# adamgreig/basebandboard

Hardware: AMD Instinct MI355X
Metric: awgn_clt_gsamples_per_s (higher is better)
Workload: dtype u32 bit-sliced GF(2) / int8 out

## Files before the change

### basebandboard_amd/csrc/awgn_kernels.hip

```cpp
#include "bbb_common.hpp"
#include "bitslice_util.hpp"
#include "awgn_launch.hpp"

#include <cstdlib>
#include <mutex>
#include <type_traits>
#include "gen/lutopt256_gen.inc"

namespace bbb {


template <int W32, typename TabPtr>
__device__ __forceinline__ void nibble_matvec_part(TabPtr tab, int nlo, int nhi, const uint32_t (&x)[W32],
                                                   uint32_t (&y)[W32]) {
    constexpr int C = (W32 % 4 == 0) ? 4 : (W32 % 2 == 0 ? 2 : 1);
    constexpr int NC = W32 / C;
    typedef uint32_t chunk_t __attribute__((ext_vector_type(C)));
#pragma unroll
    for (int w = 0; w < W32; w++) {
        uint32_t xw = x[w];
        asm volatile("" : "+v"(xw));
#pragma unroll
        for (int q = 0; q < 8; q += 2) {
            const int n0 = w * 8 + q, n1 = n0 + 1;
// ... 368 lines not shown


struct TxFuse {
    int16_t coeffs[64];
    const uint32_t *bits;
    uint32_t rel_base;
    uint32_t c0;
    int32_t noise_var;
    int32_t bit_en;
    int32_t use_bits;
    uint32_t last_word;
};

static TxFuse make_txfuse(const int16_t *coeffs, const uint32_t *d_bits, uint32_t nwords32, uint32_t rel_base, uint32_t c0, int noise_var,
                          int bit_en, int use_bits) {
    TxFuse tx;
    for (int i = 0; i < 64; i++) tx.coeffs[i] = coeffs[i];
    tx.bits = d_bits;
    tx.rel_base = rel_base;
    tx.c0 = c0;
    tx.noise_var = noise_var;
    tx.bit_en = bit_en;
    tx.use_bits = use_bits && nwords32 >= 2;
    tx.last_word = nwords32 ? nwords32 - 1 : 1;
    return tx;
}

__device__ __forceinline__ uint32_t bfi_uniform(uint32_t mask, uint32_t a, uint32_t b) {
    uint32_t d;
    asm("v_bfi_b32 %0, %1, %2, %3" : "=v"(d) : "s"(mask), "v"(a), "v"(b));
    return d;
}

typedef uint16_t u16x2 __attribute__((ext_vector_type(2)));
typedef int16_t i16x2 __attribute__((ext_vector_type(2)));

template <bool TX>
__global__ void __launch_bounds__(64) __attribute__((amdgpu_waves_per_eu(1, 1)))
awgn256_kernel(const uint32_t *__restrict planes, void *__restrict dst_, unsigned long long nsamples,
               unsigned L, unsigned long long G, unsigned nlanes, TxFuse tx) {
    __shared__ uint32_t Z[16 * 8 * 64];
    __shared__ __attribute__((aligned(16))) uint16_t TT[TX ? 256 * 8 : 8];
    const unsigned lane = threadIdx.x;
    const unsigned long long wave = blockIdx.x;
    const unsigned long long LG = wave * 64 + lane;
    __builtin_amdgcn_s_setprio(3);

    uint32_t selmask[4] = {0, 0, 0, 0};
    if (TX) {
        for (int e = (int)lane; e < 256 * 8; e += 64) {
            const int q = e >> 3, j = e & 7, ph = (int)((tx.c0 + (unsigned)j) & 7u);
            int sum = 0;
#pragma unroll
            for (int idx = 0; idx < 8; idx++) {
                const int c = tx.coeffs[8 * idx + ph];
                sum += ((q >> (7 - idx)) & 1) ? c : -c;
            }
            const int shaped = tx.bit_en ? ((int)((unsigned)sum << 20) >> 20) : 0;
            TT[e] = (uint16_t)((unsigned)((shaped - 128 * tx.noise_var) * 16) & 0xffffu);
        }
#pragma unroll
        for (int d = 0; d < 4; d++)
            selmask[d] = (tx.c0 + 2u * (unsigned)d < 8u ? 0x0000ffffu : 0u) | (tx.c0 + 2u * (unsigned)d + 1u < 8u ? 0xffff0000u : 0u);
        __syncthreads();
    }

// ... 122 lines not shown
                        if (ii < 3) load_z(4 * ihalf + ii + 1, zn);
                        const uint32_t w4[4] = {win[ii], win[4 + ii], win[8 + ii], win[12 + ii]};
                        round_end(full_c, 4 * ihalf + ii, w4, zc);
                    }
                }
            } else {
                const uint32_t none[4] = {0, 0, 0, 0};
                uint32_t zc[16], zn[16];
                load_z(0, zn);
#pragma unroll 1
                for (unsigned i = 0; i < 8; i++) {
#pragma unroll
                    for (int e = 0; e < 16; e++) zc[e] = zn[e];
                    load_z((i + 1) & 7, zn);
                    round_end(full_c, i, none, zc);
                }
            }
        };
        if (wave_full) all_iterations(std::true_type{});
        else all_iterations(std::false_type{});
    }
}

template <bool SMALL>
__global__ void __launch_bounds__(64) __attribute__((amdgpu_waves_per_eu(1, 1)))
awgn256_planes_kernel(const uint32_t *__restrict planes, u32x4 *__restrict stage, unsigned L, unsigned nlanes
) {
    const unsigned lane = threadIdx.x;
    const unsigned long long wave = blockIdx.x;
    const unsigned long long LG = wave * 64 + lane;
    __builtin_amdgcn_s_setprio(3);
    uint32_t a[256], b[256], pa[256], pb[256], cnt[8];
    if constexpr (SMALL) {
#ifdef BBB_SMALL_THROTTLE
        asm volatile("" ::: BBB_SMALL_THROTTLE);
#endif
        const uint32_t voff = (uint32_t)LG * 4u;
#define BBB_PLANE(p) (*reinterpret_cast<const uint32_t *>(reinterpret_cast<const char *>(planes + (size_t)(p) * nlanes) + (unsigned long long)voff))
#define BBB_PARK(p) { const uint32_t v_ = BBB_PLANE(p); BBB_ACC_WRITE(pa[p], v_); }
        LUTOPT256_FOR_PARKED_HI(BBB_PARK)
#undef BBB_PARK
#pragma unroll
        for (int p = 0; p < 256; p++)
            if (!lutopt256_hi_is_parked(p)) a[p] = BBB_PLANE(p);
#undef BBB_PLANE
    } else {
#pragma unroll
        for (int p = 0; p < 256; p++) b[p] = planes[(size_t)p * nlanes + LG];
        lutopt256_advance(b, a);
#define BBB_PARK(p) BBB_ACC_WRITE(pa[p], a[p]);
        LUTOPT256_FOR_PARKED_HI(BBB_PARK)
#undef BBB_PARK
    }
    u32x4 *out = stage + (wave * L) * 128 + lane;
#pragma unroll 1
    for (unsigned t = 0; t < L; t += 2) {
        lutopt256_step_parked_hi(a, pa, b, pb, cnt);
        {
        __builtin_nontemporal_store((u32x4){cnt[0], cnt[1], cnt[2], cnt[3]}, out);
        __builtin_nontemporal_store((u32x4){cnt[4], cnt[5], cnt[6], cnt[7]}, out + 64);
        }
        lutopt256_step_parked_hi(b, pb, a, pa, cnt);
        {
        __builtin_nontemporal_store((u32x4){cnt[0], cnt[1], cnt[2], cnt[3]}, out + 128);
        __builtin_nontemporal_store((u32x4){cnt[4], cnt[5], cnt[6], cnt[7]}, out + 192);
        }
        out += 256;
    }
}

int awgn256_planes_launch(const uint32_t *d_planes, void *stage, unsigned L, unsigned nlanes, hipStream_t st, bool small_footprint) {
    if (L & 1) return fail(BBB_EINVAL, "segment length must be even");
    if (small_footprint)
        hipLaunchKernelGGL(awgn256_planes_kernel<true>, dim3(nlanes / 64), dim3(64), 0, st, d_planes, (u32x4 *)stage, L, nlanes);
    else
        hipLaunchKernelGGL(awgn256_planes_kernel<false>, dim3(nlanes / 64), dim3(64), 0, st, d_planes, (u32x4 *)stage, L, nlanes);
    BBB_HIP(hipGetLastError());
    return BBB_OK;
}

constexpr unsigned kUnplaneRaw = 32 * 1024, kUnplaneLds = 3 * 32 * 1024, kUnplaneLdsTx = kUnplaneLds + 32 * 1024 + 2 * 2048;

struct UnplaneGeom {
    unsigned w_lo, ngroups, nunits;
    unsigned per_block;
};

template <bool TXM, bool NOWRAP = false>
__global__ void __launch_bounds__(256, 7)
unplane_kernel(const u32x4 *__restrict stage, char *__restrict dst, unsigned long long win_lo, unsigned long long nbytes_, unsigned L,
               unsigned long long G, UnplaneGeom ge, TxFuse tx) {
    extern __shared__ __attribute__((aligned(16))) uint32_t lds[];
    typedef __attribute__((address_space(3))) void *lds_void_ptr;
    const unsigned tid = threadIdx.x, lane = tid & 63;
    const unsigned wv = (unsigned)__builtin_amdgcn_readfirstlane((int)(tid >> 6));
    if (blockIdx.x * ge.per_block >= ge.nunits) return;
    char *const dstw = dst - win_lo;
    const unsigned long long nbytes = win_lo + nbytes_;
    const unsigned l8 = tid & 7, qs = tid >> 3;
    const unsigned wr0 = l8 * 32 + ((((qs >> 2) ^ (2 * ((l8 >> 1) & 3))) << 2) | (qs & 3));
    const unsigned lq = (tid >> 3) & 7, c2 = tid & 7;
    const unsigned rd0 = (wv * 8 + lq) * 32 + ((c2 ^ (2 * ((lq >> 1) & 3))) << 2);
    uint32_t *const tile = lds + 2 * (kUnplaneRaw / 4);
    uint32_t *const T10 = lds + kUnplaneLds / 4;
    uint32_t *const winb = lds + kUnplaneLds / 4 + 8192;
    if (TXM) {
        uint16_t *const TT = reinterpret_cast<uint16_t *>(tile);
        for (int e = (int)tid; e < 256 * 8; e += 256) {
            const int q = e >> 3, j = e & 7, ph = (int)((tx.c0 + (unsigned)j) & 7u);
            int sum = 0;
#pragma unroll
            for (int idx = 0; idx < 8; idx++) {
                const int c = tx.coeffs[8 * idx + ph];
                sum += ((q >> (7 - idx)) & 1) ? c : -c;
            }
            const int shaped = tx.bit_en ? ((int)((unsigned)sum << 20) >> 20) : 0;
            TT[e] = (uint16_t)((unsigned)((shaped - 128 * tx.noise_var) * (NOWRAP ? 1 : 16)) & 0xffffu);
        }
        __syncthreads();
        for (unsigned p = tid; p < 1024 * 8; p += 256) {
            const unsigned q10 = p >> 3, e = 2 * (p & 7);
            const uint32_t lo = TT[(((q10 >> ((tx.c0 + e) >> 3)) & 0xffu) << 3) + (e & 7)];
            const uint32_t hi = TT[(((q10 >> ((tx.c0 + e + 1) >> 3)) & 0xffu) << 3) + ((e + 1) & 7)];
            T10[p] = lo | (hi << 16);
        }
        __syncthreads();
    }
    struct Pos { unsigned q8, rg, w; };
    auto advance = [&](Pos &p) {
        if (++p.rg == ge.ngroups) {
            p.rg = 0;
            if (++p.q8 == 8) { p.q8 = 0; p.w++; }
        }
    };
    const unsigned voff_lane = (lane & 7) * 16 + (lane >> 3) * 8192;
    auto dma_unit = [&](const Pos &p, unsigned buf) {
        const unsigned step0 = p.rg * 128;
        const unsigned long long wabs = (unsigned long long)ge.w_lo + p.w;
        const char *const sb = reinterpret_cast<const char *>(stage) + ((wabs * L + step0) * 128 + p.q8 * 8) * 16;
        uint32_t *const rawb = lds + buf * (kUnplaneRaw / 4) + wv * 8 * 256;
        if (step0 + 128 <= L) {
            const char *const pl = sb + wv * 2048 + voff_lane;
#pragma unroll
            for (unsigned k = 0; k < 8; k++)
                __builtin_amdgcn_global_load_lds((const void *)(pl + ((k & 3) * 32 * 2048 + (k >> 2) * 1024)),
                                                 (lds_void_ptr)(uintptr_t)(rawb + k * 256), 16, 0, 0);
        } else {
            const unsigned last = L - 1 - step0;
#pragma unroll
            for (unsigned k = 0; k < 8; k++) {
                unsigned st = 4 * ((k & 3) * 8 + (lane >> 3)) + wv;
                st = st < last ? st : last;
                __builtin_amdgcn_global_load_lds((const void *)(sb + (size_t)st * 2048 + (k >> 2) * 1024 + (lane & 7) * 16),
                                                 (lds_void_ptr)(uintptr_t)(rawb + k * 256), 16, 0, 0);
            }
        }
        if (TXM) {
            const long long so = (long long)((wabs * 2048 + p.q8 * 8) * (unsigned long long)L + step0) - (long long)win_lo;
#pragma unroll
            for (unsigned i = 0; i < 2; i++) {
                const unsigned e = (wv * 2 + i) * 64 + lane, row = e >> 1;
                const long long pu = so + (long long)((unsigned long long)((row >> 3) * 64 + (row & 7)) * L);
                uint32_t word = 0;
                if (pu > -128 && pu < (long long)nbytes_) word = (((uint32_t)(pu >> 3) + tx.rel_base) >> 5) + (e & 1);
                word = word < tx.last_word ? word : tx.last_word;
                __builtin_amdgcn_global_load_lds((const void *)(tx.bits + word), (lds_void_ptr)(uintptr_t)(winb + buf * 512 + (wv * 2 + i) * 64), 4, 0, 0);
            }
        }
    };
    auto wait_vm = [](unsigned n) {
        switch (n) {
#define BBB_W(N) case N: asm volatile("s_waitcnt vmcnt(" #N ")" ::: "memory"); break;
            BBB_W(8) BBB_W(10) BBB_W(16) BBB_W(26)
#undef BBB_W
        default: asm volatile("s_waitcnt vmcnt(0)" ::: "memory"); break;
        }
    };
    constexpr unsigned NDMA = TXM ? 10 : 8, NST = TXM ? 16 : 8;
    const unsigned u0 = blockIdx.x * ge.per_block;
    const unsigned n_it = ge.nunits - u0 < ge.per_block ? ge.nunits - u0 : ge.per_block;
    Pos cur;
    cur.rg = u0 % ge.ngroups;
    cur.q8 = (u0 / ge.ngroups) & 7;
    cur.w = (u0 / ge.ngroups) >> 3;
    Pos nxt = cur;
    advance(nxt);
    unsigned buf = 0;
    bool fast1 = false;
    dma_unit(cur, 0);
    for (unsigned it = 0; it < n_it; it++, buf ^= 1) {
        const unsigned q8 = cur.q8, step0 = cur.rg * 128;
        const unsigned long long w = (unsigned long long)ge.w_lo + cur.w;
        const bool more1 = it + 1 < n_it;
        if (more1) dma_unit(nxt, buf ^ 1);
        wait_vm((more1 ? NDMA : 0u) + (fast1 ? NST : 0u));
        __builtin_amdgcn_s_barrier();
        {
            const uint32_t *raw = lds + buf * (kUnplaneRaw / 4) + (qs * 8 + l8) * 4;
            uint32_t Z[4][8];
#pragma unroll
            for (unsigned s = 0; s < 4; s++) {
                const u32x4 lo = *reinterpret_cast<const u32x4 *>(raw + (2 * s) * 1024);
                const u32x4 hi = *reinterpret_cast<const u32x4 *>(raw + (2 * s + 1) * 1024);
                Z[s][0] = lo[0]; Z[s][1] = lo[1]; Z[s][2] = lo[2]; Z[s][3] = lo[3];
                Z[s][4] = hi[0]; Z[s][5] = hi[1]; Z[s][6] = hi[2]; Z[s][7] = TXM ? ~hi[3] : hi[3];
            }
#pragma unroll
            for (unsigned s = 0; s < 4; s++) planes8_to_bytes(Z[s]);
#pragma unroll
            for (unsigned i = 0; i < 8; i++) {
                uint32_t z[4] = {Z[0][i], Z[1][i], Z[2][i], Z[3][i]};
                transpose4x4_bytes(z);
#pragma unroll
                for (unsigned q = 0; q < 4; q++) tile[wr0 + (8 * q + i) * 256] = z[q];
            }
        }
        asm volatile("s_waitcnt lgkmcnt(0)" ::: "memory");
        __builtin_amdgcn_s_barrier();
        const unsigned inseg = step0 + c2 * 16;
        const unsigned long long g0 = (w * 32 + wv) * 64 + q8 * 8 + lq;
        unsigned long long off = g0 * (unsigned long long)L + inseg;
        const unsigned long long goff = 256ull * L;
        const bool lane_fast = inseg < L && g0 + 7 * 256 < G && off >= win_lo && off + 7 * goff + 16 <= nbytes;
        const bool wave_fast = __all(lane_fast);
        fast1 = wave_fast;
        if (!TXM && inseg < L) {
            if (wave_fast) {
#pragma unroll
                for (unsigned k = 0; k < 8; k++) {
                    const u32x4 v = *reinterpret_cast<const u32x4 *>(&tile[rd0 + k * 1024]);
                    *reinterpret_cast<u32x4 *>(dstw + off) = v;
                    off += goff;
                }
            } else {
                for (unsigned k = 0; k < 8; k++, off += goff) {
                    if (g0 + 256ull * k >= G || off >= nbytes) break;
                    if (off < win_lo) continue;
                    const u32x4 v = *reinterpret_cast<const u32x4 *>(&tile[rd0 + k * 1024]);
// ... 36 lines not shown
                        x[2 * w4] = __builtin_bit_cast(uint32_t, __builtin_bit_cast(i16x2, m01) >> 4);
                        x[2 * w4 + 1] = __builtin_bit_cast(uint32_t, __builtin_bit_cast(i16x2, m23) >> 4);
                    }
                }
                int16_t *out = dst16 + (o - win_lo);
                if (FULL || o + 16 <= nbytes) {
                    const u32x4 lo = {x[0], x[1], x[2], x[3]}, hi = {x[4], x[5], x[6], x[7]};
                    reinterpret_cast<u32x4 *>(out)[0] = lo;
                    reinterpret_cast<u32x4 *>(out)[1] = hi;
                } else {
                    const unsigned n = (unsigned)(nbytes - o);
                    for (unsigned e = 0; e < n; e++) out[e] = (int16_t)((x[e >> 1] >> (16 * (e & 1))) & 0xffff);
                }
            };
            if (wave_fast) {
#pragma unroll 1
                for (unsigned k4 = 0; k4 < 8; k4 += 4) {
#pragma unroll
                    for (unsigned k = 0; k < 4; k++) piece(std::true_type{}, k4 + k, off + (k4 + k) * goff);
                }
            } else {
#pragma unroll 1
                for (unsigned k = 0; k < 8; k++) {
                    const unsigned long long o = off + k * goff;
                    if (g0 + 256ull * k >= G || o >= nbytes) break;
                    if (o < win_lo) continue;
                    piece(std::false_type{}, k, o);
                }
            }
        }
        asm volatile("s_waitcnt lgkmcnt(0)" ::: "memory");
        __builtin_amdgcn_s_barrier();
        cur = nxt;
        advance(nxt);
    }
}

static bool unplane_tx_nowrap(const TxFuse &tx) {
    int worst = 0;
    if (tx.bit_en)
        for (int ph = 0; ph < 8; ph++) {
            int sum = 0;
            for (int idx = 0; idx < 8; idx++) sum += tx.coeffs[8 * idx + ph] < 0 ? -(int)tx.coeffs[8 * idx + ph] : (int)tx.coeffs[8 * idx + ph];
            worst = sum > worst ? sum : worst;
        }
    return tx.noise_var >= 0 && worst + 128 * tx.noise_var <= 2047;
}

static int unplane_launch_with(const void *stage, void *dst, uint64_t win_lo, uint64_t nbytes, unsigned L, uint64_t G, unsigned nlanes,
                               const TxFuse *tx, hipStream_t st) {
    if (win_lo & 15) return fail(BBB_EINVAL, "window must start on a 16-byte boundary of the staged stream");
    if (nbytes == 0) return BBB_OK;
    int dev = 0, ncu = 256;
    BBB_HIP(hipGetDevice(&dev));
    BBB_HIP(hipDeviceGetAttribute(&ncu, hipDeviceAttributeMultiprocessorCount, dev));
    const uint64_t seg = (uint64_t)L * 2048;
    const unsigned w_lo = (unsigned)(win_lo / seg);
    uint64_t w_hi = (win_lo + nbytes + seg - 1) / seg;
    if (w_hi > nlanes / 64) w_hi = nlanes / 64;
    const unsigned w_n = (unsigned)(w_hi - w_lo);
    const unsigned ngroups = (L + 127) / 128;
    const uint64_t nunits = (uint64_t)w_n * ngroups * 8;
    if (nunits >> 32) return fail(BBB_EINVAL, "staged window too large for one mover launch (2^32 units of 32 KiB)");
    uint64_t blocks = (uint64_t)ncu * (uint64_t)env_knob("BBB_UNPLANE_BLOCKS_PER_CU", 1);
    if (blocks > nunits) blocks = nunits;
    UnplaneGeom ge;
    ge.w_lo = w_lo; ge.ngroups = ngroups; ge.nunits = (unsigned)nunits;
    ge.per_block = (unsigned)((nunits + blocks - 1) / blocks);
    blocks = (nunits + ge.per_block - 1) / ge.per_block;
    {
        static std::mutex mu;
        static bool attr_set[64] = {false};
        std::lock_guard<std::mutex> g(mu);
        if (dev < 0 || dev >= 64 || !attr_set[dev]) {
            BBB_HIP(hipFuncSetAttribute((const void *)unplane_kernel<false>, hipFuncAttributeMaxDynamicSharedMemorySize, (int)kUnplaneLds));
            BBB_HIP(hipFuncSetAttribute((const void *)unplane_kernel<true>, hipFuncAttributeMaxDynamicSharedMemorySize, (int)kUnplaneLdsTx));
            BBB_HIP(hipFuncSetAttribute((const void *)unplane_kernel<true, true>, hipFuncAttributeMaxDynamicSharedMemorySize, (int)kUnplaneLdsTx));
            if (dev >= 0 && dev < 64) attr_set[dev] = true;
        }
    }
    if (tx && unplane_tx_nowrap(*tx)) {
        hipLaunchKernelGGL((unplane_kernel<true, true>), dim3((unsigned)blocks), dim3(256), kUnplaneLdsTx, st, (const u32x4 *)stage, (char *)dst,
                           (unsigned long long)win_lo, (unsigned long long)nbytes, L, (unsigned long long)G, ge, *tx);
    } else if (tx) {
        hipLaunchKernelGGL(unplane_kernel<true>, dim3((unsigned)blocks), dim3(256), kUnplaneLdsTx, st, (const u32x4 *)stage, (char *)dst,
                           (unsigned long long)win_lo, (unsigned long long)nbytes, L, (unsigned long long)G, ge, *tx);
    } else {
        TxFuse none{};
        hipLaunchKernelGGL(unplane_kernel<false>, dim3((unsigned)blocks), dim3(256), kUnplaneLds, st, (const u32x4 *)stage, (char *)dst,
                           (unsigned long long)win_lo, (unsigned long long)nbytes, L, (unsigned long long)G, ge, none);
    }
    BBB_HIP(hipGetLastError());
    return BBB_OK;
}

int unplane_launch(const void *stage, void *dst, uint64_t win_lo, uint64_t nbytes, unsigned L, uint64_t G, unsigned nlanes, hipStream_t st) {
    return unplane_launch_with(stage, dst, win_lo, nbytes, L, G, nlanes, nullptr, st);
}

int unplane_tx_launch(const void *stage, int16_t *dst, uint64_t win_lo, uint64_t nsamples, unsigned L, uint64_t G, unsigned nlanes,
// ... 406 lines not shown
```

### basebandboard_amd/csrc/awgn_launch.hpp

```cpp
#pragma once
#include "bbb_common.hpp"

namespace bbb {

int awgn_seed_launch(int k, const uint32_t *d_tabs, const uint32_t *s16, uint64_t G, uint32_t *d_states,
                     uint64_t stride, unsigned nlanes, uint32_t *d_planes, hipStream_t st, int slice_mode = 0, int parts = 2);
constexpr int kSeedTopTables = 31;
struct PrbsSeedRide { int k; const uint32_t *d_tabs, *s16, *qcol; unsigned nlanes; uint32_t *d_planes; };
int awgn_seed_head_launch(int k, const uint32_t *d_tabs, const uint32_t *s16, uint64_t G, uint32_t *d_states, hipStream_t st,
                          const PrbsSeedRide *ride = nullptr);
int awgn_seed_tail_planes_launch(int k, const uint32_t *d_top, uint64_t G, const uint32_t *d_states, unsigned nlanes, uint32_t *d_planes,
                                 hipStream_t st);
int prbs_seed_planes_launch(int k, const uint32_t *d_tabs, const uint32_t *s16, uint64_t G, uint32_t *d_states, unsigned nlanes,
                            uint32_t *d_planes, hipStream_t st);
int prbs_seed_lanes_launch(int k, const uint32_t *d_tabs, const uint32_t *s16, const uint32_t *qcol, uint64_t G, unsigned nlanes,
                           uint32_t *d_planes, hipStream_t st);
bool awgn512p_matches(int k, const uint16_t *taps, const uint32_t *row_off);
int bitslice512p_launch(const uint32_t *d_states, uint64_t G, uint64_t stride, unsigned nlanes, uint32_t *d_planes, hipStream_t st);
int awgn512p_fill_launch(const uint32_t *d_planes, int16_t *dst, uint64_t nsamples, unsigned L, uint64_t G, unsigned nlanes,
                         hipStream_t st);
int awgn256_fill_launch(const uint32_t *d_planes, int8_t *dst, uint64_t nsamples, unsigned L, uint64_t G,
                        unsigned nlanes, hipStream_t st);
int awgn256_planes_launch(const uint32_t *d_planes, void *stage, unsigned L, unsigned nlanes, hipStream_t st, bool small_footprint);
int unplane_launch(const void *stage, void *dst, uint64_t win_lo, uint64_t nbytes, unsigned L, uint64_t G, unsigned nlanes, hipStream_t st);
int unplane_tx_launch(const void *stage, int16_t *dst, uint64_t win_lo, uint64_t nsamples, unsigned L, uint64_t G, unsigned nlanes,
                      const int16_t *coeffs, const uint32_t *d_bits, uint32_t nwords32, uint32_t rel_base, uint32_t c0, int noise_var, int bit_en,
                      int use_bits, hipStream_t st);
int awgn256_tx_launch(const uint32_t *d_planes, int16_t *dst, uint64_t nsamples, unsigned L, uint64_t G, unsigned nlanes,
                      const int16_t *coeffs, const uint32_t *d_bits, uint32_t nwords32, uint32_t rel_base, uint32_t c0, int noise_var,
                      int bit_en, int use_bits, hipStream_t st);
int pulse_bits_launch(uint64_t *dst, int64_t m_first, uint64_t nwords, hipStream_t st);
int widen_i8_i16_launch(const int8_t *src, int16_t *dst, uint64_t n, hipStream_t st);
int awgn_generic_fill_launch(int k, const uint16_t *d_taps, const uint32_t *d_row_off, uint32_t *d_planes2,
                             void *dst, int elem_size, uint64_t nsamples, unsigned L, uint64_t G, unsigned nlanes,
                             hipStream_t st);
int lutopt_words_launch(int k, const uint16_t *d_taps, const uint32_t *d_row_off, uint32_t *d_planes2, uint32_t *dst,
                        uint64_t nstates, unsigned L, uint64_t G, unsigned nlanes, bool msb_first, hipStream_t st);
int lutopt_words256_launch(const uint32_t *d_planes, uint32_t *dst, uint64_t nstates, unsigned L, uint64_t G, unsigned nlanes,
                           bool msb_first, hipStream_t st);
int clt_tree_launch(int k, const uint64_t *states, uint64_t nstates, int16_t *out, hipStream_t st);
bool awgn256_matches(int k, const uint16_t *taps, const uint32_t *row_off);
int awgn_small_matches(int k, const uint16_t *taps, const uint32_t *row_off);
int awgn_small_fill_launch(int k, const uint32_t *d_planes, int8_t *dst, uint64_t nsamples, unsigned L, uint64_t G,
                           unsigned nlanes, hipStream_t st);

struct TrialDev {
    int32_t prbs_k, prbs_tap;
    int32_t nthr[2];
    int32_t thr[2][4];
    uint32_t L;
    uint64_t G, nbits;
    uint32_t flags, last_len;
};
enum { kTrialLastLen = 1, kTrialSaveState = 2 };
#define BBB_BER_MAX_GROUP 12
// ... 13 lines not shown
```

### basebandboard_amd/csrc/bbb_api.hip

```cpp
#include "bbb_common.hpp"
#include "awgn_launch.hpp"
#include "gf2.hpp"
#include "rccl_loader.hpp"
#include "sweep_shard.hpp"
#include "sweep_threads.hpp"

#include <algorithm>
#include <cstdlib>
#include <cstring>
#include <map>
#include <memory>
#include <mutex>
#include <thread>
#include <utility>
#include <vector>

namespace bbb {

std::string &last_error() {
    static thread_local std::string s;
    return s;
}

int use_device(int device) {
// ... 437 lines not shown
    hipEvent_t m0 = nullptr, m1 = nullptr;
    if (h->profiling) {
        BBB_HIP(hipEventCreate(&m0)); BBB_HIP(hipEventCreate(&m1));
        BBB_HIP(hipEventRecord(m0, ms));
    }
    if ((rc = launch_mover((const void *)h->d_stage[slot].p, ms))) return rc;
    if (h->profiling) {
        BBB_HIP(hipEventRecord(m1, ms));
        h->prof_mover_pending.emplace_back(m0, m1);
    }
    if ((rc = h->stage_free[slot].record(ms))) return rc;
    h->stage_busy[slot] = true;
    h->stage_gen[slot]++;
    if (own_stream) BBB_HIP(hipStreamWaitEvent(h->stream, h->stage_free[slot], 0));
    return BBB_OK;
}

bbb_lutopt::Ahead take_ahead(bbb_lutopt *h) {
    const bbb_lutopt::Ahead a = h->ahead;
    h->ahead.first += a.n; h->ahead.step += a.n;
    h->ahead.win_lo += a.n;
    h->ahead.valid = --h->ahead.left > 0;
    return a;
}

int deliver_i8(bbb_lutopt *h, int slot, void *dst, uint64_t win_lo, uint64_t n, uint64_t L, uint64_t G, unsigned nlanes) {
    return queue_mover_with(h, slot, [&](const void *stage, hipStream_t ys) {
        return unplane_launch(stage, dst, win_lo, n, (unsigned)L, G, nlanes, ys);
    });
}

int produce_planes(bbb_lutopt *h, uint64_t L, unsigned nlanes, bbb_lutopt::ProfEv *ev, bool planes_seeded_after_mover, int *slot_out,
                   bool small_footprint = false) {
    const size_t need_words = (size_t)nlanes * (size_t)L * 8;
    const int slot = h->stage_slot ^= 1;
    *slot_out = slot;
    if (h->ahead.valid && h->ahead.slot == slot) h->ahead.valid = false;
    int rc;
    if (h->d_stage[slot].cap < need_words) {
        if (h->stage_busy[slot]) BBB_HIP(hipEventSynchronize(h->stage_free[slot]));
        h->stage_busy[slot] = false;
        if ((rc = h->d_stage[slot].grow(need_words))) return rc;
    }
    const bool seeding_saw_last_mover = planes_seeded_after_mover && h->pf_waited_slot == slot && h->pf_waited_gen == h->stage_gen[slot];
    if (planes_seeded_after_mover) h->pf_waited_slot = -1;
    if (h->stage_busy[slot] && !seeding_saw_last_mover)
        BBB_HIP(hipStreamWaitEvent(h->cs, h->stage_free[slot], 0));
    if (ev) BBB_HIP(hipEventRecord(ev->e1, h->cs));
    rc = awgn256_planes_launch(h->cur.buf[kPlanes], (void *)h->d_stage[slot].p, (unsigned)L, nlanes, h->cs, small_footprint);
    h->last_staged_small = small_footprint;
    if (rc) return rc;
    if ((rc = mark_planes_read(h))) return rc;
    if (ev) BBB_HIP(hipEventRecord(ev->e2, h->cs));
    return h->stage_arith[slot].record(h->cs);
}

bool partition512(const bbb_lutopt *h, uint64_t nsamples, uint64_t *L, uint64_t *G, unsigned *nlanes) {
    const uint64_t gmax = (uint64_t)h->max_waves * 1024;
    uint64_t l = (nsamples + gmax - 1) / gmax;
    if (l < 64) l = 64;
    l = (l + 7) / 8 * 8;
    if (l > 0xffffff00ull) return false;
    *L = l;
    *G = (nsamples + l - 1) / l;
    *nlanes = (unsigned)((*G + 1023) / 1024 * 64);
    return true;
}
// ... 1414 lines not shown
```

### basebandboard_amd/csrc/bitslice_util.hpp

```cpp
#pragma once
#include <cstdint>

#ifndef BBB_HD
#ifdef __HIPCC__
#define BBB_HD __host__ __device__ __forceinline__
#else
#define BBB_HD inline
#endif
#endif

namespace bbb {

BBB_HD void transpose32(uint32_t (&q)[32]) {
#define BBB_T32_STAGE(S, M)                                         \
    _Pragma("unroll") for (int i = 0; i < 32; i++) {                \
        if ((i & (S)) == 0) {                                       \
            const uint32_t t = ((q[i] >> (S)) ^ q[i + (S)]) & (M);  \
            q[i + (S)] ^= t;                                        \
            q[i] ^= t << (S);                                       \
        }                                                           \
    }
    BBB_T32_STAGE(16, 0x0000FFFFu)
    BBB_T32_STAGE(8, 0x00FF00FFu)
    BBB_T32_STAGE(4, 0x0F0F0F0Fu)
// ... 11 lines not shown
    for (int i = 0; i < 4; i++) r |= (uint32_t)((in >> (8 * ((sel >> (8 * i)) & 7))) & 0xff) << (8 * i);
    return r;
#endif
}

BBB_HD uint32_t bit_select(uint32_t mask, uint32_t a, uint32_t b) { return (mask & a) | (~mask & b); }

BBB_HD void planes8_to_bytes(uint32_t (&c)[8]) {
#define BBB_B8_STAGE(S, M)                                              \
    _Pragma("unroll") for (int i = 0; i < 8; i++) {                     \
        if ((i & (S)) == 0) {                                           \
            const uint32_t x = c[i], y = c[i + (S)];                    \
            c[i] = bit_select((M), x, y << (S));                        \
            c[i + (S)] = bit_select((M), x >> (S), y);                  \
        }                                                               \
    }
    BBB_B8_STAGE(4, 0x0F0F0F0Fu)
    BBB_B8_STAGE(2, 0x33333333u)
    BBB_B8_STAGE(1, 0x55555555u)
#undef BBB_B8_STAGE
}

BBB_HD void transpose4x4_bytes(uint32_t (&r)[4]) {
    const uint32_t a = byte_perm(r[1], r[0], 0x05010400u);
    const uint32_t b = byte_perm(r[1], r[0], 0x07030602u);
    const uint32_t c = byte_perm(r[3], r[2], 0x05010400u);
    const uint32_t d = byte_perm(r[3], r[2], 0x07030602u);
    r[0] = byte_perm(c, a, 0x05040100u);
    r[1] = byte_perm(c, a, 0x07060302u);
    r[2] = byte_perm(d, b, 0x05040100u);
    r[3] = byte_perm(d, b, 0x07060302u);
}

BBB_HD uint64_t gen_index(uint64_t wave, unsigned lane, unsigned j) { return (wave * 32 + j) * 64 + lane; }

constexpr uint64_t kThueMorse64 = 0x9669699669969669ull;

}
```

### basebandboard_amd/csrc/hist_kernels.hip

```cpp
#include "bbb_common.hpp"
#include "bitslice_util.hpp"

#include <algorithm>
#include <mutex>

namespace bbb {

typedef uint32_t hist_u32x4 __attribute__((ext_vector_type(4)));

constexpr unsigned kHistLanes = 64;
constexpr unsigned kHistRaw = 32 * 1024;
constexpr unsigned kHistTable = 256 * kHistLanes * 4;
constexpr unsigned kHistPlanesLds = kHistTable + 2 * kHistRaw;
constexpr int kHistSampleThreads = 1024;

struct HistGeom {
    unsigned ngroups, nunits;
    unsigned per_block;
};

__device__ __forceinline__ uint32_t hist_fold(const uint32_t *H, unsigned bin) {
    uint32_t sum = 0;
    for (unsigned l = 0; l < kHistLanes; l++) sum += H[bin * kHistLanes + ((l + bin) & (kHistLanes - 1))];
    return sum;
}

__global__ void __launch_bounds__(256, 7)
hist_planes_kernel(const hist_u32x4 *__restrict stage, unsigned long long nsamples, unsigned L, HistGeom ge, uint32_t *__restrict scratch) {
    extern __shared__ __attribute__((aligned(16))) uint32_t lds[];
    typedef __attribute__((address_space(3))) void *lds_void_ptr;
    const unsigned tid = threadIdx.x, lane = tid & 63;
    const unsigned wv = (unsigned)__builtin_amdgcn_readfirstlane((int)(tid >> 6));
    uint32_t *const H = lds;
    uint32_t *const raw0 = lds + kHistTable / 4;
    {
        hist_u32x4 *h4 = reinterpret_cast<hist_u32x4 *>(H);
        for (unsigned i = tid; i < kHistTable / 16; i += 256) h4[i] = hist_u32x4{0u, 0u, 0u, 0u};
    }
    __syncthreads();
    const unsigned l8 = tid & 7, qs = tid >> 3;
    const uint32_t hbase = (uint32_t)(uintptr_t)(lds_void_ptr)H;
    const uint32_t column = lane * 4u;
    struct Pos { unsigned q8, rg, w; };
    auto advance = [&](Pos &p) {
        if (++p.rg == ge.ngroups) {
            p.rg = 0;
            if (++p.q8 == 8) { p.q8 = 0; p.w++; }
        }
    };
    const unsigned voff_lane = (lane & 7) * 16 + (lane >> 3) * 8192;
    auto dma_unit = [&](const Pos &p, unsigned buf) {
        const unsigned step0 = p.rg * 128;
        const char *const sb = reinterpret_cast<const char *>(stage) + (((unsigned long long)p.w * L + step0) * 128 + p.q8 * 8) * 16;
        uint32_t *const rawb = raw0 + buf * (kHistRaw / 4) + wv * 8 * 256;
        if (step0 + 128 <= L) {
            const char *const pl = sb + wv * 2048 + voff_lane;
#pragma unroll
            for (unsigned k = 0; k < 8; k++)
                __builtin_amdgcn_global_load_lds((const void *)(pl + ((k & 3) * 32 * 2048 + (k >> 2) * 1024)),
                                                 (lds_void_ptr)(uintptr_t)(rawb + k * 256), 16, 0, 0);
        } else {
            const unsigned last = L - 1 - step0;
#pragma unroll
            for (unsigned k = 0; k < 8; k++) {
                unsigned st = 4 * ((k & 3) * 8 + (lane >> 3)) + wv;
                st = st < last ? st : last;
                __builtin_amdgcn_global_load_lds((const void *)(sb + (size_t)st * 2048 + (k >> 2) * 1024 + (lane & 7) * 16),
                                                 (lds_void_ptr)(uintptr_t)(rawb + k * 256), 16, 0, 0);
            }
        }
    };
    const unsigned u0 = blockIdx.x * ge.per_block;
    const unsigned n_it = u0 >= ge.nunits ? 0u : (ge.nunits - u0 < ge.per_block ? ge.nunits - u0 : ge.per_block);
    Pos cur;
    cur.rg = u0 % ge.ngroups;
    cur.q8 = (u0 / ge.ngroups) & 7;
    cur.w = (u0 / ge.ngroups) >> 3;
    Pos nxt = cur;
    advance(nxt);
    unsigned buf = 0;
    if (n_it) dma_unit(cur, 0);
    for (unsigned it = 0; it < n_it; it++, buf ^= 1) {
        const bool more = it + 1 < n_it;
        if (more) dma_unit(nxt, buf ^ 1);
        if (more) asm volatile("s_waitcnt vmcnt(8)" ::: "memory");
        else asm volatile("s_waitcnt vmcnt(0)" ::: "memory");
        __builtin_amdgcn_s_barrier();
        {
            const uint32_t *raw = raw0 + buf * (kHistRaw / 4) + (qs * 8 + l8) * 4;
            uint32_t Z[4][8];
#pragma unroll
            for (unsigned s = 0; s < 4; s++) {
                const hist_u32x4 lo = *reinterpret_cast<const hist_u32x4 *>(raw + (2 * s) * 1024);
                const hist_u32x4 hi = *reinterpret_cast<const hist_u32x4 *>(raw + (2 * s + 1) * 1024);
                Z[s][0] = lo[0]; Z[s][1] = lo[1]; Z[s][2] = lo[2]; Z[s][3] = lo[3];
                Z[s][4] = hi[0]; Z[s][5] = hi[1]; Z[s][6] = hi[2]; Z[s][7] = ~hi[3];
            }
#pragma unroll
            for (unsigned s = 0; s < 4; s++) planes8_to_bytes(Z[s]);
            const unsigned step = cur.rg * 128 + 4 * qs;
            const unsigned long long span = 64ull * L;
            const unsigned long long off0 = ((unsigned long long)cur.w * 2048 + cur.q8 * 8 + l8) * L + step;
#define BBB_HIST_ADD(WORD, Q) \
    asm volatile("ds_add_u32 %0, %1" ::"v"(hbase + __builtin_amdgcn_perm(column, (WORD), 0x0c0c0004u | ((Q) << 8))), "v"(1u) : "memory")
            if (step + 3 < L && off0 + 3 + 31 * span < nsamples) {
#pragma unroll
                for (unsigned s = 0; s < 4; s++) {
#pragma unroll
                    for (unsigned i = 0; i < 8; i++) {
                        BBB_HIST_ADD(Z[s][i], 0u); BBB_HIST_ADD(Z[s][i], 1u); BBB_HIST_ADD(Z[s][i], 2u); BBB_HIST_ADD(Z[s][i], 3u);
                    }
                }
            } else {
#pragma unroll
                for (unsigned s = 0; s < 4; s++) {
                    const unsigned long long o = off0 + s;
                    unsigned nj = 0;
                    if (step + s < L && o < nsamples) {
                        const unsigned long long m = (nsamples - o - 1) / span + 1;
                        nj = m < 32 ? (unsigned)m : 32u;
                    }
#pragma unroll
                    for (unsigned i = 0; i < 8; i++) {
                        if (i < nj) BBB_HIST_ADD(Z[s][i], 0u);
                        if (i + 8 < nj) BBB_HIST_ADD(Z[s][i], 1u);
                        if (i + 16 < nj) BBB_HIST_ADD(Z[s][i], 2u);
                        if (i + 24 < nj) BBB_HIST_ADD(Z[s][i], 3u);
                    }
                }
            }
#undef BBB_HIST_ADD
        }
        asm volatile("s_waitcnt lgkmcnt(0)" ::: "memory");
        __builtin_amdgcn_s_barrier();
        cur = nxt;
        advance(nxt);
    }
    __syncthreads();
    scratch[(size_t)blockIdx.x * 256 + tid] = hist_fold(H, tid);
}

template <typename T>
__global__ void __launch_bounds__(kHistSampleThreads)
hist_samples_kernel(const T *__restrict x, unsigned long long nsamples, unsigned nbins, uint32_t *__restrict scratch) {
    extern __shared__ __attribute__((aligned(16))) uint32_t lds[];
    uint32_t *const H = lds;
    for (unsigned i = threadIdx.x; i < nbins * kHistLanes; i += kHistSampleThreads) H[i] = 0u;
    __syncthreads();
    constexpr unsigned PER = 16 / sizeof(T);
    const unsigned lane = threadIdx.x & 63, half = nbins >> 1, mask = nbins - 1;
    const unsigned long long ngroups = nsamples / PER;
    const hist_u32x4 *xv = reinterpret_cast<const hist_u32x4 *>(x);
    const unsigned long long stride = (unsigned long long)gridDim.x * kHistSampleThreads;
    for (unsigned long long g = (unsigned long long)blockIdx.x * kHistSampleThreads + threadIdx.x; g < ngroups; g += stride) {
        const hist_u32x4 v = xv[g];
#pragma unroll
        for (unsigned e = 0; e < PER; e++) {
            int s;
            if (sizeof(T) == 1) s = (int)(int8_t)((v[e >> 2] >> (8 * (e & 3))) & 0xffu);
            else s = (int)(int16_t)((v[e >> 1] >> (16 * (e & 1))) & 0xffffu);
            atomicAdd(&H[(((unsigned)s + half) & mask) * kHistLanes + lane], 1u);
        }
    }
    if (blockIdx.x == 0) {
        const unsigned long long i = ngroups * PER + threadIdx.x;
        if (threadIdx.x < PER && i < nsamples) atomicAdd(&H[(((unsigned)(int)x[i] + half) & mask) * kHistLanes + lane], 1u);
    }
    __syncthreads();
    for (unsigned bin = threadIdx.x; bin < nbins; bin += kHistSampleThreads) scratch[(size_t)blockIdx.x * nbins + bin] = hist_fold(H, bin);
// ... 9 lines not shown
}

int hist_grid_blocks() {
    int dev = 0, cus = 0;
    BBB_HIP(hipGetDevice(&dev));
    BBB_HIP(hipDeviceGetAttribute(&cus, hipDeviceAttributeMultiprocessorCount, dev));
    return std::max(cus, 1);
}

static int hist_lds_attributes() {
    static std::mutex mu;
    static bool attr_set[64] = {false};
    int dev = 0;
    BBB_HIP(hipGetDevice(&dev));
    std::lock_guard<std::mutex> g(mu);
    if (dev < 0 || dev >= 64 || !attr_set[dev]) {
        const int most = (int)(kHistMaxBins * kHistLanes * 4);
        BBB_HIP(hipFuncSetAttribute((const void *)hist_planes_kernel, hipFuncAttributeMaxDynamicSharedMemorySize, (int)kHistPlanesLds));
        BBB_HIP(hipFuncSetAttribute((const void *)hist_samples_kernel<int8_t>, hipFuncAttributeMaxDynamicSharedMemorySize, most));
        BBB_HIP(hipFuncSetAttribute((const void *)hist_samples_kernel<int16_t>, hipFuncAttributeMaxDynamicSharedMemorySize, most));
        if (dev >= 0 && dev < 64) attr_set[dev] = true;
    }
    return BBB_OK;
}

int hist_planes_launch(const void *stage, uint64_t nsamples, unsigned L, unsigned nlanes, uint32_t *scratch, int blocks, unsigned *used,
                       hipStream_t st) {
    if (nsamples == 0 || nsamples > (1ull << 31)) return fail(BBB_EINVAL, "a histogram launch counts 1 .. 2^31 samples");
    if (L == 0 || blocks < 1) return fail(BBB_EINVAL, "bad histogram launch");
    const uint64_t seg = (uint64_t)L * 2048;
    const uint64_t w_n = std::min<uint64_t>((nsamples + seg - 1) / seg, nlanes / 64);
    HistGeom ge;
    ge.ngroups = (L + 127) / 128;
    const uint64_t nunits = w_n * ge.ngroups * 8;
    if (nunits == 0 || nunits >> 32) return fail(BBB_EINVAL, "staged range out of the histogram mover's reach");
    ge.nunits = (unsigned)nunits;
    const uint64_t want = std::min<uint64_t>((uint64_t)blocks, nunits);
    ge.per_block = (unsigned)((nunits + want - 1) / want);
    const unsigned nb = (unsigned)((nunits + ge.per_block - 1) / ge.per_block);
    int rc = hist_lds_attributes();
    if (rc) return rc;
    hipLaunchKernelGGL(hist_planes_kernel, dim3(nb), dim3(256), kHistPlanesLds, st, (const hist_u32x4 *)stage, (unsigned long long)nsamples, L, ge,
                       scratch);
    BBB_HIP(hipGetLastError());
    *used = nb;
    return BBB_OK;
}

int hist_samples_launch(const void *samples, int elem, uint64_t nsamples, unsigned nbins, uint32_t *scratch, int blocks, unsigned *used,
                        hipStream_t st) {
    if (nsamples == 0 || nsamples > (1ull << 31)) return fail(BBB_EINVAL, "a histogram launch counts 1 .. 2^31 samples");
    if (nbins < 2 || nbins > kHistMaxBins || (nbins & (nbins - 1)) || blocks < 1 || ((uintptr_t)samples & 15) || (elem != 1 && elem != 2))
        return fail(BBB_EINVAL, "bad histogram launch");
    int rc = hist_lds_attributes();
    if (rc) return rc;
    const uint64_t want = (nsamples + (uint64_t)kHistSampleThreads * 256 - 1) / ((uint64_t)kHistSampleThreads * 256);
    const unsigned nb = (unsigned)std::max<uint64_t>(1, std::min<uint64_t>(want, (uint64_t)blocks));
    const size_t smem = (size_t)nbins * kHistLanes * 4;
    if (elem == 1)
        hipLaunchKernelGGL(hist_samples_kernel<int8_t>, dim3(nb), dim3(kHistSampleThreads), smem, st, (const int8_t *)samples,
                           (unsigned long long)nsamples, nbins, scratch);
    else
        hipLaunchKernelGGL(hist_samples_kernel<int16_t>, dim3(nb), dim3(kHistSampleThreads), smem, st, (const int16_t *)samples,
                           (unsigned long long)nsamples, nbins, scratch);
    BBB_HIP(hipGetLastError());
    *used = nb;
// ... 12 lines not shown
```

Before: 969.5.

## Compress staged plane counts by eliding redundant high planes with per-step tail flags

```diff
diff --git a/basebandboard_amd/csrc/awgn_kernels.hip b/basebandboard_amd/csrc/awgn_kernels.hip
--- a/basebandboard_amd/csrc/awgn_kernels.hip
+++ b/basebandboard_amd/csrc/awgn_kernels.hip
@@ -424,6 +424,7 @@
     return d;
 }
 
+typedef uint32_t u32x2 __attribute__((ext_vector_type(2)));
 typedef uint16_t u16x2 __attribute__((ext_vector_type(2)));
 typedef int16_t i16x2 __attribute__((ext_vector_type(2)));
 
@@ -612,9 +613,6 @@
     __builtin_amdgcn_s_setprio(3);
     uint32_t a[256], b[256], pa[256], pb[256], cnt[8];
     if constexpr (SMALL) {
-#ifdef BBB_SMALL_THROTTLE
-        asm volatile("" ::: BBB_SMALL_THROTTLE);
-#endif
         const uint32_t voff = (uint32_t)LG * 4u;
 #define BBB_PLANE(p) (*reinterpret_cast<const uint32_t *>(reinterpret_cast<const char *>(planes + (size_t)(p) * nlanes) + (unsigned long long)voff))
 #define BBB_PARK(p) { const uint32_t v_ = BBB_PLANE(p); BBB_ACC_WRITE(pa[p], v_); }
@@ -632,21 +630,44 @@
         LUTOPT256_FOR_PARKED_HI(BBB_PARK)
 #undef BBB_PARK
     }
-    u32x4 *out = stage + (wave * L) * 128 + lane;
+    char *out = reinterpret_cast<char *>(stage + (wave * L) * 128);
+    uint32_t *const flagw = reinterpret_cast<uint32_t *>(stage + (unsigned long long)gridDim.x * L * 128) + wave * stage6_flag_words(L);
+    const uint32_t voff_a = lane * 16u, voff_b = 1024u + lane * 8u;
+    uint32_t tails = 0;
+#define BBB_STAGE_STEP(OFF, BIT)                                                                                                    \
+    {                                                                                                                               \
+        const u32x4 a_ = {cnt[0], cnt[1], cnt[2], cnt[3]};                                                                          \
+        const u32x2 lo_ = {cnt[4], cnt[7]}, hi_ = {cnt[5], cnt[6]};                                                                 \
+        const uint32_t m_ = (cnt[5] ^ cnt[7]) | (cnt[6] ^ cnt[7]);                                                                  \
+        asm volatile("global_store_dwordx4 %[va], %[a], %[sb] offset:%[oa] nt\n\t"                                                  \
+                     "global_store_dwordx2 %[vb], %[lo], %[sb] offset:%[oa] nt\n\t"                                                 \
+                     "v_cmp_ne_u32_e32 vcc, 0, %[m]\n\t"                                                                            \
+                     "s_cbranch_vccz .Lbbb_notail_%=\n\t"                                                                           \
+                     "global_store_dwordx2 %[vb], %[hi], %[sb] offset:%[ob] nt\n\t"                                                 \
+                     "s_bitset1_b32 %[acc], %[bit]\n"                                                                               \
+                     ".Lbbb_notail_%=:"                                                                                             \
+                     : [acc] "+s"(tails)                                                                                            \
+                     : [m] "v"(m_), [va] "v"(voff_a), [vb] "v"(voff_b), [a] "v"(a_), [lo] "v"(lo_), [hi] "v"(hi_), [sb] "s"(out),   \
+                       [oa] "n"(OFF), [ob] "n"((OFF) + 512), [bit] "s"(BIT)                                                         \
+                     : "vcc", "memory");                                                                                            \
+    }
 #pragma unroll 1
-    for (unsigned t = 0; t < L; t += 2) {
-        lutopt256_step_parked_hi(a, pa, b, pb, cnt);
-        {
-        __builtin_nontemporal_store((u32x4){cnt[0], cnt[1], cnt[2], cnt[3]}, out);
-        __builtin_nontemporal_store((u32x4){cnt[4], cnt[5], cnt[6], cnt[7]}, out + 64);
-        }
-        lutopt256_step_parked_hi(b, pb, a, pa, cnt);
-        {
-        __builtin_nontemporal_store((u32x4){cnt[0], cnt[1], cnt[2], cnt[3]}, out + 128);
-        __builtin_nontemporal_store((u32x4){cnt[4], cnt[5], cnt[6], cnt[7]}, out + 192);
-        }
-        out += 256;
-    }
+    for (unsigned t0 = 0; t0 < L; t0 += 32) {
+        const unsigned t1 = t0 + 32 < L ? t0 + 32 : L;
+#pragma unroll 1
+        for (unsigned t = t0; t < t1; t += 2) {
+            lutopt256_step_parked_hi(a, pa, b, pb, cnt);
+            BBB_STAGE_STEP(0, t)
+            lutopt256_step_parked_hi(b, pb, a, pa, cnt);
+            BBB_STAGE_STEP(2048, t + 1)
+            out += 4096;
+        }
+        uint32_t tv_;
+        asm volatile("v_mov_b32 %0, %1\n\ts_mov_b32 %1, 0" : "=v"(tv_), "+s"(tails));
+        if (lane == 0) flagw[t0 >> 5] = tv_;
+    }
+#undef BBB_STAGE_STEP
+    if (lane < stage6_flag_words(L) - (L + 31) / 32) flagw[(L + 31) / 32 + lane] = 0u;
 }
 
 int awgn256_planes_launch(const uint32_t *d_planes, void *stage, unsigned L, unsigned nlanes, hipStream_t st, bool small_footprint) {
@@ -664,6 +685,7 @@
 struct UnplaneGeom {
     unsigned w_lo, ngroups, nunits;
     unsigned per_block;
+    unsigned nwaves;
 };
 
 template <bool TXM, bool NOWRAP = false>
@@ -713,28 +735,12 @@
             if (++p.q8 == 8) { p.q8 = 0; p.w++; }
         }
     };
-    const unsigned voff_lane = (lane & 7) * 16 + (lane >> 3) * 8192;
-    auto dma_unit = [&](const Pos &p, unsigned buf) {
+    const Stage6Slot slot = stage6_slot(stage, ge.nwaves, L);
+    auto unit_flags = [&](const Pos &p) { return stage6_unit_flags(slot, (unsigned long long)ge.w_lo + p.w, p.rg); };
+    auto dma_unit = [&](const Pos &p, unsigned buf, stage6_u32x4 fl) {
         const unsigned step0 = p.rg * 128;
         const unsigned long long wabs = (unsigned long long)ge.w_lo + p.w;
-        const char *const sb = reinterpret_cast<const char *>(stage) + ((wabs * L + step0) * 128 + p.q8 * 8) * 16;
-        uint32_t *const rawb = lds + buf * (kUnplaneRaw / 4) + wv * 8 * 256;
-        if (step0 + 128 <= L) {
-            const char *const pl = sb + wv * 2048 + voff_lane;
-#pragma unroll
-            for (unsigned k = 0; k < 8; k++)
-                __builtin_amdgcn_global_load_lds((const void *)(pl + ((k & 3) * 32 * 2048 + (k >> 2) * 1024)),
-                                                 (lds_void_ptr)(uintptr_t)(rawb + k * 256), 16, 0, 0);
-        } else {
-            const unsigned last = L - 1 - step0;
-#pragma unroll
-            for (unsigned k = 0; k < 8; k++) {
-                unsigned st = 4 * ((k & 3) * 8 + (lane >> 3)) + wv;
-                st = st < last ? st : last;
-                __builtin_amdgcn_global_load_lds((const void *)(sb + (size_t)st * 2048 + (k >> 2) * 1024 + (lane & 7) * 16),
-                                                 (lds_void_ptr)(uintptr_t)(rawb + k * 256), 16, 0, 0);
-            }
-        }
+        stage6_dma_unit(slot, wabs, p.q8, p.rg, fl, lds + buf * (kUnplaneRaw / 4), wv, lane);
         if (TXM) {
             const long long so = (long long)((wabs * 2048 + p.q8 * 8) * (unsigned long long)L + step0) - (long long)win_lo;
 #pragma unroll
@@ -756,7 +762,7 @@
         default: asm volatile("s_waitcnt vmcnt(0)" ::: "memory"); break;
         }
     };
-    constexpr unsigned NDMA = TXM ? 10 : 8, NST = TXM ? 16 : 8;
+    constexpr unsigned NDMA = kStage6Dma + (TXM ? 2 : 0), NST = TXM ? 16 : 8;
     const unsigned u0 = blockIdx.x * ge.per_block;
     const unsigned n_it = ge.nunits - u0 < ge.per_block ? ge.nunits - u0 : ge.per_block;
     Pos cur;
@@ -767,23 +773,24 @@
     advance(nxt);
     unsigned buf = 0;
     bool fast1 = false;
-    dma_unit(cur, 0);
+    stage6_u32x4 fl_cur = unit_flags(cur), fl_nxt = unit_flags(nxt);
+    dma_unit(cur, 0, fl_cur);
     for (unsigned it = 0; it < n_it; it++, buf ^= 1) {
         const unsigned q8 = cur.q8, step0 = cur.rg * 128;
         const unsigned long long w = (unsigned long long)ge.w_lo + cur.w;
         const bool more1 = it + 1 < n_it;
-        if (more1) dma_unit(nxt, buf ^ 1);
+        if (more1) dma_unit(nxt, buf ^ 1, fl_nxt);
+        Pos nn = nxt;
+        advance(nn);
+        const stage6_u32x4 fl_nn = unit_flags(nn);
         wait_vm((more1 ? NDMA : 0u) + (fast1 ? NST : 0u));
         __builtin_amdgcn_s_barrier();
         {
-            const uint32_t *raw = lds + buf * (kUnplaneRaw / 4) + (qs * 8 + l8) * 4;
             uint32_t Z[4][8];
-#pragma unroll
-            for (unsigned s = 0; s < 4; s++) {
-                const u32x4 lo = *reinterpret_cast<const u32x4 *>(raw + (2 * s) * 1024);
-                const u32x4 hi = *reinterpret_cast<const u32x4 *>(raw + (2 * s + 1) * 1024);
-                Z[s][0] = lo[0]; Z[s][1] = lo[1]; Z[s][2] = lo[2]; Z[s][3] = lo[3];
-                Z[s][4] = hi[0]; Z[s][5] = hi[1]; Z[s][6] = hi[2]; Z[s][7] = TXM ? ~hi[3] : hi[3];
+            stage6_load_planes(lds + buf * (kUnplaneRaw / 4), qs, l8, wv, fl_cur, Z);
+            if (TXM) {
+#pragma unroll
+                for (unsigned s = 0; s < 4; s++) Z[s][7] = ~Z[s][7];
             }
 #pragma unroll
             for (unsigned s = 0; s < 4; s++) planes8_to_bytes(Z[s]);
@@ -886,7 +893,9 @@
         asm volatile("s_waitcnt lgkmcnt(0)" ::: "memory");
         __builtin_amdgcn_s_barrier();
         cur = nxt;
-        advance(nxt);
+        nxt = nn;
+        fl_cur = fl_nxt;
+        fl_nxt = fl_nn;
     }
 }
 
@@ -919,7 +928,7 @@
     uint64_t blocks = (uint64_t)ncu * (uint64_t)env_knob("BBB_UNPLANE_BLOCKS_PER_CU", 1);
     if (blocks > nunits) blocks = nunits;
     UnplaneGeom ge;
-    ge.w_lo = w_lo; ge.ngroups = ngroups; ge.nunits = (unsigned)nunits;
+    ge.w_lo = w_lo; ge.ngroups = ngroups; ge.nunits = (unsigned)nunits; ge.nwaves = nlanes / 64;
     ge.per_block = (unsigned)((nunits + blocks - 1) / blocks);
     blocks = (nunits + ge.per_block - 1) / ge.per_block;
     {
diff --git a/basebandboard_amd/csrc/awgn_launch.hpp b/basebandboard_amd/csrc/awgn_launch.hpp
--- a/basebandboard_amd/csrc/awgn_launch.hpp
+++ b/basebandboard_amd/csrc/awgn_launch.hpp
@@ -21,6 +21,10 @@
                          hipStream_t st);
 int awgn256_fill_launch(const uint32_t *d_planes, int8_t *dst, uint64_t nsamples, unsigned L, uint64_t G,
                         unsigned nlanes, hipStream_t st);
+constexpr inline unsigned stage6_flag_words(uint64_t L) { return (unsigned)((L + 127) / 128 * 4); }
+constexpr inline size_t awgn256_stage_words(unsigned nlanes, uint64_t L) {
+    return (size_t)nlanes * (size_t)L * 8 + (size_t)(nlanes / 64) * stage6_flag_words(L);
+}
 int awgn256_planes_launch(const uint32_t *d_planes, void *stage, unsigned L, unsigned nlanes, hipStream_t st, bool small_footprint);
 int unplane_launch(const void *stage, void *dst, uint64_t win_lo, uint64_t nbytes, unsigned L, uint64_t G, unsigned nlanes, hipStream_t st);
 int unplane_tx_launch(const void *stage, int16_t *dst, uint64_t win_lo, uint64_t nsamples, unsigned L, uint64_t G, unsigned nlanes,
diff --git a/basebandboard_amd/csrc/bbb_api.hip b/basebandboard_amd/csrc/bbb_api.hip
--- a/basebandboard_amd/csrc/bbb_api.hip
+++ b/basebandboard_amd/csrc/bbb_api.hip
@@ -493,7 +493,7 @@
 
 int produce_planes(bbb_lutopt *h, uint64_t L, unsigned nlanes, bbb_lutopt::ProfEv *ev, bool planes_seeded_after_mover, int *slot_out,
                    bool small_footprint = false) {
-    const size_t need_words = (size_t)nlanes * (size_t)L * 8;
+    const size_t need_words = awgn256_stage_words(nlanes, L);
     const int slot = h->stage_slot ^= 1;
     *slot_out = slot;
     if (h->ahead.valid && h->ahead.slot == slot) h->ahead.valid = false;
diff --git a/basebandboard_amd/csrc/bitslice_util.hpp b/basebandboard_amd/csrc/bitslice_util.hpp
--- a/basebandboard_amd/csrc/bitslice_util.hpp
+++ b/basebandboard_amd/csrc/bitslice_util.hpp
@@ -67,6 +67,82 @@
     r[3] = byte_perm(d, b, 0x07060302u);
 }
 
+#if defined(__HIPCC__)
+typedef uint32_t stage6_u32x4 __attribute__((ext_vector_type(4)));
+typedef uint32_t stage6_u32x2 __attribute__((ext_vector_type(2)));
+constexpr unsigned kStage6RawWords = 8192;
+constexpr unsigned kStage6Dma = 8;
+
+struct Stage6Slot {
+    const char *rows;
+    const stage6_u32x4 *flags;
+    unsigned L, ngroups;
+    unsigned long long nflags;
+};
+
+__device__ __forceinline__ Stage6Slot stage6_slot(const void *stage, unsigned nwaves, unsigned L) {
+    Stage6Slot sl;
+    sl.rows = reinterpret_cast<const char *>(stage);
+    sl.flags = reinterpret_cast<const stage6_u32x4 *>(sl.rows + (unsigned long long)nwaves * L * 2048);
+    sl.L = L;
+    sl.ngroups = (L + 127) / 128;
+    sl.nflags = (unsigned long long)nwaves * sl.ngroups;
+    return sl;
+}
+
+__device__ __forceinline__ stage6_u32x4 stage6_unit_flags(const Stage6Slot &sl, unsigned long long w, unsigned rg) {
+    unsigned long long i = w * sl.ngroups + rg;
+    i = i < sl.nflags ? i : sl.nflags - 1;
+    typedef const __attribute__((address_space(4))) stage6_u32x4 *const_ptr;
+    return *(const_ptr)(uintptr_t)(sl.flags + i);
+}
+
+__device__ __forceinline__ void stage6_dma_unit(const Stage6Slot &sl, unsigned long long w, unsigned q8, unsigned rg, stage6_u32x4 fl,
+                                                uint32_t *raw, unsigned wv, unsigned lane) {
+    typedef __attribute__((address_space(3))) void *lds_void_ptr;
+    asm volatile("" : "+v"(lane));
+    const unsigned step0 = rg * 128;
+    const char *const sb = sl.rows + (w * sl.L + step0) * 2048;
+    const char *const idle = reinterpret_cast<const char *>(sl.flags);
+    uint32_t *const raw_a = raw + wv * 1024, *const raw_lo = raw + 4096 + wv * 512, *const raw_hi = raw + 6144 + wv * 512;
+    const unsigned last = sl.L - 1 - step0;
+    const bool whole = step0 + 128 <= sl.L;
+    const unsigned pos_a = 4 * (lane >> 3) + wv, pos_b = 4 * (lane >> 2) + wv;
+    const unsigned in_a = q8 * 128 + (lane & 7) * 16, in_b = 1024 + q8 * 64 + (lane & 3) * 16;
+    auto step_of = [&](unsigned pos) { return whole ? pos : (pos < last ? pos : last); };
+#pragma unroll
+    for (unsigned k = 0; k < 4; k++)
+        __builtin_amdgcn_global_load_lds((const void *)(sb + (size_t)step_of(pos_a + 32 * k) * 2048 + in_a),
+                                         (lds_void_ptr)(uintptr_t)(raw_a + k * 256), 16, 0, 0);
+#pragma unroll
+    for (unsigned k = 0; k < 2; k++)
+        __builtin_amdgcn_global_load_lds((const void *)(sb + (size_t)step_of(pos_b + 64 * k) * 2048 + in_b),
+                                         (lds_void_ptr)(uintptr_t)(raw_lo + k * 256), 16, 0, 0);
+#pragma unroll
+    for (unsigned k = 0; k < 2; k++) {
+        const uint32_t fw = (lane & 32) ? fl[2 * k + 1] : fl[2 * k];
+        const bool tail = (fw >> (pos_b & 31)) & 1u;
+        const char *const src = sb + (size_t)step_of(pos_b + 64 * k) * 2048 + in_b + 512;
+        __builtin_amdgcn_global_load_lds((const void *)(tail ? src : idle), (lds_void_ptr)(uintptr_t)(raw_hi + k * 256), 16, 0, 0);
+    }
+}
+
+__device__ __forceinline__ void stage6_load_planes(const uint32_t *raw, unsigned qs, unsigned l8, unsigned wv, stage6_u32x4 fl,
+                                                   uint32_t (&Z)[4][8]) {
+    const uint32_t fw = (wv == 0 ? fl[0] : wv == 1 ? fl[1] : wv == 2 ? fl[2] : fl[3]) >> (4 * (qs & 7));
+    const uint32_t *const pa = raw + (qs * 8 + l8) * 4, *const pb = raw + 4096 + (qs * 8 + l8) * 2;
+#pragma unroll
+    for (unsigned s = 0; s < 4; s++) {
+        const stage6_u32x4 a = *reinterpret_cast<const stage6_u32x4 *>(pa + s * 1024);
+        const stage6_u32x2 lo = *reinterpret_cast<const stage6_u32x2 *>(pb + s * 512);
+        const stage6_u32x2 hi = *reinterpret_cast<const stage6_u32x2 *>(pb + 2048 + s * 512);
+        const bool tail = (fw >> s) & 1u;
+        Z[s][0] = a[0]; Z[s][1] = a[1]; Z[s][2] = a[2]; Z[s][3] = a[3];
+        Z[s][4] = lo[0]; Z[s][5] = tail ? hi[0] : lo[1]; Z[s][6] = tail ? hi[1] : lo[1]; Z[s][7] = lo[1];
+    }
+}
+#endif
+
 BBB_HD uint64_t gen_index(uint64_t wave, unsigned lane, unsigned j) { return (wave * 32 + j) * 64 + lane; }
 
 constexpr uint64_t kThueMorse64 = 0x9669699669969669ull;
diff --git a/basebandboard_amd/csrc/hist_kernels.hip b/basebandboard_amd/csrc/hist_kernels.hip
--- a/basebandboard_amd/csrc/hist_kernels.hip
+++ b/basebandboard_amd/csrc/hist_kernels.hip
@@ -6,7 +6,7 @@
 
 namespace bbb {
 
-typedef uint32_t hist_u32x4 __attribute__((ext_vector_type(4)));
+typedef stage6_u32x4 hist_u32x4;
 
 constexpr unsigned kHistLanes = 64;
 constexpr unsigned kHistRaw = 32 * 1024;
@@ -17,6 +17,7 @@
 struct HistGeom {
     unsigned ngroups, nunits;
     unsigned per_block;
+    unsigned nwaves;
 };
 
 __device__ __forceinline__ uint32_t hist_fold(const uint32_t *H, unsigned bin) {
@@ -48,27 +49,10 @@
             if (++p.q8 == 8) { p.q8 = 0; p.w++; }
         }
     };
-    const unsigned voff_lane = (lane & 7) * 16 + (lane >> 3) * 8192;
-    auto dma_unit = [&](const Pos &p, unsigned buf) {
-        const unsigned step0 = p.rg * 128;
-        const char *const sb = reinterpret_cast<const char *>(stage) + (((unsigned long long)p.w * L + step0) * 128 + p.q8 * 8) * 16;
-        uint32_t *const rawb = raw0 + buf * (kHistRaw / 4) + wv * 8 * 256;
-        if (step0 + 128 <= L) {
-            const char *const pl = sb + wv * 2048 + voff_lane;
-#pragma unroll
-            for (unsigned k = 0; k < 8; k++)
-                __builtin_amdgcn_global_load_lds((const void *)(pl + ((k & 3) * 32 * 2048 + (k >> 2) * 1024)),
-                                                 (lds_void_ptr)(uintptr_t)(rawb + k * 256), 16, 0, 0);
-        } else {
-            const unsigned last = L - 1 - step0;
-#pragma unroll
-            for (unsigned k = 0; k < 8; k++) {
-                unsigned st = 4 * ((k & 3) * 8 + (lane >> 3)) + wv;
-                st = st < last ? st : last;
-                __builtin_amdgcn_global_load_lds((const void *)(sb + (size_t)st * 2048 + (k >> 2) * 1024 + (lane & 7) * 16),
-                                                 (lds_void_ptr)(uintptr_t)(rawb + k * 256), 16, 0, 0);
-            }
-        }
+    const Stage6Slot slot = stage6_slot(stage, ge.nwaves, L);
+    auto unit_flags = [&](const Pos &p) { return stage6_unit_flags(slot, p.w, p.rg); };
+    auto dma_unit = [&](const Pos &p, unsigned buf, stage6_u32x4 fl) {
+        stage6_dma_unit(slot, p.w, p.q8, p.rg, fl, raw0 + buf * (kHistRaw / 4), wv, lane);
     };
     const unsigned u0 = blockIdx.x * ge.per_block;
     const unsigned n_it = u0 >= ge.nunits ? 0u : (ge.nunits - u0 < ge.per_block ? ge.nunits - u0 : ge.per_block);
@@ -79,23 +63,23 @@
     Pos nxt = cur;
     advance(nxt);
     unsigned buf = 0;
-    if (n_it) dma_unit(cur, 0);
+    stage6_u32x4 fl_cur = unit_flags(cur), fl_nxt = unit_flags(nxt);
+    if (n_it) dma_unit(cur, 0, fl_cur);
     for (unsigned it = 0; it < n_it; it++, buf ^= 1) {
         const bool more = it + 1 < n_it;
-        if (more) dma_unit(nxt, buf ^ 1);
+        if (more) dma_unit(nxt, buf ^ 1, fl_nxt);
+        Pos nn = nxt;
+        advance(nn);
+        const stage6_u32x4 fl_nn = unit_flags(nn);
+        static_assert(kStage6Dma == 8, "the wait below counts a unit's DMA instructions");
         if (more) asm volatile("s_waitcnt vmcnt(8)" ::: "memory");
         else asm volatile("s_waitcnt vmcnt(0)" ::: "memory");
         __builtin_amdgcn_s_barrier();
         {
-            const uint32_t *raw = raw0 + buf * (kHistRaw / 4) + (qs * 8 + l8) * 4;
             uint32_t Z[4][8];
-#pragma unroll
-            for (unsigned s = 0; s < 4; s++) {
-                const hist_u32x4 lo = *reinterpret_cast<const hist_u32x4 *>(raw + (2 * s) * 1024);
-                const hist_u32x4 hi = *reinterpret_cast<const hist_u32x4 *>(raw + (2 * s + 1) * 1024);
-                Z[s][0] = lo[0]; Z[s][1] = lo[1]; Z[s][2] = lo[2]; Z[s][3] = lo[3];
-                Z[s][4] = hi[0]; Z[s][5] = hi[1]; Z[s][6] = hi[2]; Z[s][7] = ~hi[3];
-            }
+            stage6_load_planes(raw0 + buf * (kHistRaw / 4), qs, l8, wv, fl_cur, Z);
+#pragma unroll
+            for (unsigned s = 0; s < 4; s++) Z[s][7] = ~Z[s][7];
 #pragma unroll
             for (unsigned s = 0; s < 4; s++) planes8_to_bytes(Z[s]);
             const unsigned step = cur.rg * 128 + 4 * qs;
@@ -134,7 +118,9 @@
         asm volatile("s_waitcnt lgkmcnt(0)" ::: "memory");
         __builtin_amdgcn_s_barrier();
         cur = nxt;
-        advance(nxt);
+        nxt = nn;
+        fl_cur = fl_nxt;
+        fl_nxt = fl_nn;
     }
     __syncthreads();
     scratch[(size_t)blockIdx.x * 256 + tid] = hist_fold(H, tid);
@@ -210,6 +196,7 @@
     const uint64_t w_n = std::min<uint64_t>((nsamples + seg - 1) / seg, nlanes / 64);
     HistGeom ge;
     ge.ngroups = (L + 127) / 128;
+    ge.nwaves = nlanes / 64;
     const uint64_t nunits = w_n * ge.ngroups * 8;
     if (nunits == 0 || nunits >> 32) return fail(BBB_EINVAL, "staged range out of the histogram mover's reach");
     ge.nunits = (unsigned)nunits;
```

Result: faster. 982.6 (median of 5 runs) (+1.3%).
